# tohinz/multiple-objects-gan

Measured on AMD Instinct MI355X. Metric: images/sec per G+D train step, 256x256 coco-attngan, higher is better.
Workload: dtype f32

## Files before the change

include/mogan_hip.h:

```cpp
#ifndef MOGAN_HIP_H
#define MOGAN_HIP_H

#include <stddef.h>
#include <stdint.h>

#ifdef __cplusplus
extern "C" {
#endif

typedef struct ihipStream_t* hipStream_t;

#define MOGAN_ERR_SHAPE (-1)
#define MOGAN_ERR_LAUNCH (-2)
#define MOGAN_ERR_WS (-3)

#define MOGAN_ACT_NONE 0
#define MOGAN_ACT_RELU 1
#define MOGAN_ACT_LRELU 2
#define MOGAN_ACT_GLU 3
#define MOGAN_ACT_TANH 4
#define MOGAN_ACT_SIGMOID 5

int mogan_abi_version(void);
int mogan_gemm_set_split_target(int blocks);
// ... 34 lines not shown
typedef struct MoganConvDgradArgs {
    const float* dy; long long dy_bstride; const float* w; float* dx; long long dx_bstride;
    const float* relu_of; long long relu_bstride; int accumulate;
    int B, Cin, Hs, Ws, Cout, KH, KW, stride, ph, pw;
} MoganConvDgradArgs;
int mogan_conv2d_affine_fwd_group(int n, const MoganConvFwdArgs* args, void* ws, size_t ws_bytes, hipStream_t stream);
int mogan_conv2d_dgrad_group(int n, const MoganConvDgradArgs* args, void* ws, size_t ws_bytes, hipStream_t stream);
int mogan_conv2d_affine_fwd_ex(const float* x, long long x_bstride, const float* w, const float* scale, const float* shift,
                               float* y, long long y_bstride, float* y2, long long y2_bstride, int msplit, int B, int Cin,
                               int Hs, int Ws, int Cout, int KH, int KW, int stride, int ph, int pw, int relu, void* ws,
                               size_t ws_bytes, hipStream_t stream);
int mogan_conv2d_fwd_ex(const float* x, long long x_bstride, const float* w, float* y, long long y_bstride,
                        const float* relu_of, long long relu_bstride, int accumulate, int B, int Cin, int Hs, int Ws,
                        int Cout, int KH, int KW, int stride, int ph, int pw, void* ws, size_t ws_bytes, hipStream_t stream);
int mogan_conv2d_dgrad_ex(const float* dy, long long dy_bstride, const float* w, float* dx, long long dx_bstride,
                          const float* relu_of, long long relu_bstride, int accumulate, int B, int Cin, int Hs, int Ws,
                          int Cout, int KH, int KW, int stride, int ph, int pw, void* ws, size_t ws_bytes,
                          hipStream_t stream);
int mogan_conv2d_dgrad(const float* dy, const float* w, float* dx, int B, int Cin, int Hs, int Ws, int Cout, int KH,
                       int KW, int stride, int ph, int pw, int up, void* ws, size_t ws_bytes, hipStream_t stream);
size_t mogan_wino_prep_bytes(int B, int Cin, int Hs, int Ws, int Cout, int KH, int KW, int stride, int ph, int pw, int up, int dgrad);
int mogan_wino_prep_group(int n, const float* const* w, void* const* prep, const int* Cout, const int* Cin, const int* dgrad,
                          hipStream_t stream);
size_t mogan_conv_prep_bytes(int B, int Cin, int Hs, int Ws, int Cout, int KH, int KW, int stride, int ph, int pw, int up, int dgrad);
int mogan_conv_prep_group(int n, const float* const* w, void* const* prep, const int* Cout, const int* Cin, const int* KH,
                          const int* dgrad, hipStream_t stream);
int mogan_conv2d_fwd_wp(const float* x, const float* w, const void* wprep, float* y, int B, int Cin, int Hs, int Ws, int Cout, int KH,
                        int KW, int stride, int ph, int pw, int up, void* ws, size_t ws_bytes, hipStream_t stream);
int mogan_conv2d_dgrad_wp(const float* dy, const float* w, const void* wprep, float* dx, int B, int Cin, int Hs, int Ws, int Cout,
                          int KH, int KW, int stride, int ph, int pw, int up, void* ws, size_t ws_bytes, hipStream_t stream);
int mogan_conv2d_wgrad(const float* dy, const float* x, float* dw, int B, int Cin, int Hs, int Ws, int Cout, int KH,
                       int KW, int stride, int ph, int pw, int up, int accumulate, void* ws, size_t ws_bytes,
                       hipStream_t stream);

int mogan_pk_conv_eligible(int B, int Cin, int Hs, int Ws, int Cout, int KH, int KW, int stride, int ph, int pw, int dgrad);
size_t mogan_pk_weight_bytes(int Cout, int Cin, int KH, int KW, int stride, int dgrad);
int mogan_pk_weight_pack(const float* w, void* wpk, int Cout, int Cin, int KH, int KW, int stride, int ph, int pw, int dgrad,
                         hipStream_t stream);
int mogan_pk_weight_pack_both(const float* w, void* wpk_fwd, void* wpk_dgrad, int Cout, int Cin, int KH, int KW, int stride, int ph,
                              int pw, hipStream_t stream);
int mogan_conv2d_fwd_pk(const float* x, const void* wpk, float* y, int B, int Cin, int Hs, int Ws, int Cout, int KH, int KW,
                        int stride, int ph, int pw, void* ws, size_t ws_bytes, hipStream_t stream);
int mogan_conv2d_dgrad_pk(const float* dy, const void* wpk, float* dx, int B, int Cin, int Hs, int Ws, int Cout, int KH, int KW,
                          int stride, int ph, int pw, void* ws, size_t ws_bytes, hipStream_t stream);
int mogan_pk_debug_force(int take_all, int cfg, int split);
int mogan_pk_wgrad_eligible(int B, int Cin, int Hs, int Ws, int Cout, int KH, int KW, int stride, int ph, int pw, size_t ws_bytes);
int mogan_conv2d_wgrad_pk(const float* dy, const float* x, float* dw, int B, int Cin, int Hs, int Ws, int Cout, int KH, int KW,
                          int stride, int ph, int pw, int accumulate, void* ws, size_t ws_bytes, hipStream_t stream);

size_t mogan_pk_panel_bytes(int B, int C, int HW);
int mogan_deep_block_eligible(int B, int Cin, int Hs, int Ws, int Cout, int KH, int KW, int stride, int ph, int pw, int act,
                              int groups);
int mogan_deep_conv_bn_act_fwd(const float* x, const void* xpanel, const void* wpk, const float* gamma, const float* beta,
                               float* rmean, float* rvar, float* y, float* stats, float* z, void* zpanel, int B, int Cin, int Hs,
                               int Ws, int Cout, int KH, int KW, int stride, int ph, int pw, float eps, float momentum, int act,
                               float slope, int groups, void* ws, size_t ws_bytes, hipStream_t stream);
int mogan_deep_conv_bn_act_bwd(const float* dz, const float* y, const float* stats, const float* gamma, const float* beta,
                               const void* wpk_dgrad, float* dy, float* dgamma, float* dbeta, int accumulate, float* dx, int B,
                               int Cin, int Hs, int Ws, int Cout, int KH, int KW, int stride, int ph, int pw, int act, float slope,
                               int groups, void* ws, size_t ws_bytes, hipStream_t stream);

typedef struct MoganPkArgs {
    const void* wpk; const void* panel; float* raw;
    int B, M;
    int Cp, CGp, cg0;
    int PH, PW, outH, outW;
// ... 219 lines not shown
```

multiple-objects-gan_amd/csrc/mogan_dconv2.hip:

```cpp
#include <hip/hip_runtime.h>
#include <stdint.h>
#include <stdlib.h>
#include <algorithm>
#include "../../include/mogan_hip.h"
#include "mogan_internal.h"
#include "mogan_mma.h"

#if MOGAN_X6
#if defined(DCONV2_LAB) && DCONV2_LAB == 9
__device__ unsigned long long g_d2_seg[8];
#define D2_T(var) const unsigned long long var = __builtin_readcyclecounter()
#define D2_ADD(i, a, b) do { if (tid == 0) atomicAdd(&g_d2_seg[i], (b) - (a)); } while (0)
extern "C" int mogan_lab_d2_segments(unsigned long long* out, int reset) {
    if (hipMemcpyFromSymbol(out, HIP_SYMBOL(g_d2_seg), sizeof(g_d2_seg)) != hipSuccess) return -1;
    if (reset) { unsigned long long z[8] = {0}; if (hipMemcpyToSymbol(HIP_SYMBOL(g_d2_seg), z, sizeof(z)) != hipSuccess) return -1; }
    return 0;
}
#else
#define D2_T(var) do {} while (0)
#define D2_ADD(i, a, b) do {} while (0)
#endif
namespace {

typedef float f32x16 __attribute__((ext_vector_type(16)));
typedef float f32x4 __attribute__((ext_vector_type(4)));

__device__ __forceinline__ float ldg1(__amdgpu_buffer_rsrc_t r, unsigned idx) {
    return __builtin_bit_cast(float, __builtin_amdgcn_raw_buffer_load_b32(r, idx * 4u, 0, 0));
}
__device__ __forceinline__ f32x4 ldg4w(__amdgpu_buffer_rsrc_t r, unsigned idx) {
    return __builtin_bit_cast(f32x4, __builtin_amdgcn_raw_buffer_load_b128(r, idx * 4u, 0, 0));
}
#define D2_OOB 0x3FFFFFFFu

struct D2P {
    const float* X; const void* Wp; float* Y; float* ws;
    int B, Cin, Cout, H, W;
    int CinX;
    int OH, OW, pt, pl;
// ... 240 lines not shown
            for (int tt = 0; tt < TM; ++tt)
#pragma unroll
                for (int r = 0; r < 16; ++r) {
                    ybase[(size_t)(tt * 32 + (r & 3) + 8 * (r >> 2)) * plane] = acc[tt][r];
                    acc[tt][r] = 0.f;
                }
        } else {
#pragma unroll
            for (int tt = 0; tt < TM; ++tt)
#pragma unroll
                for (int r = 0; r < 16; ++r) {
                    const int mr = tt * 32 + (r & 3) + 8 * (r >> 2);
                    if (m0 + mr + 4 * h < p.Cout) {
                        float* dst = ybase + (size_t)mr * plane;
                        float v = acc[tt][r];
                        if (addc) v += *dst;
                        *dst = v;
                    }
                    acc[tt][r] = 0.f;
                }
        }
        D2_T(t_e1); D2_ADD(5, t_e0, t_e1);
    }
}

__global__ __launch_bounds__(256) void dconv2_reduce_kernel(const float* __restrict__ ws, float* __restrict__ out, long long n,
                                                            long long slab, int nsplit, int acc) {
    const long long i = (long long)blockIdx.x * 256 + threadIdx.x;
    if (i >= n) return;
    float s = acc ? out[i] : 0.f;
    for (int k = 0; k < nsplit; ++k) s += ws[(size_t)k * slab + i];
    out[i] = s;
}

static inline long long cdiv2(long long a, long long b) { return (a + b - 1) / b; }

template <int KH, int KW, int TM, int NS, int CW, bool S2D>
static int launch2g(D2P& p, hipStream_t st) {
    constexpr int KHW = KH * KW, NPIX = (256 / CW + KH - 1) * (CW + KW - 1);
    constexpr size_t lds = (size_t)NS * 6 * NPIX * 16 + (size_t)TM * 32 * ((size_t)NS * KHW * 6 + 1) * 16;
    static_assert(lds <= 160 * 1024, "LDS budget");
    static bool attr = false;
    if (!attr) {
        if (hipFuncSetAttribute((const void*)dconv2_fwd_kernel<KH, KW, TM, NS, CW, S2D>, hipFuncAttributeMaxDynamicSharedMemorySize,
                                (int)lds) != hipSuccess) return MOGAN_ERR_LAUNCH;
        attr = true;
    }
    dim3 grid((unsigned)cdiv2(p.ntiles, p.tpb), (unsigned)cdiv2(p.Cout, TM * 32), (unsigned)(p.nsplit * p.npar));
    hipLaunchKernelGGL((dconv2_fwd_kernel<KH, KW, TM, NS, CW, S2D>), grid, dim3(512), lds, st, p);
    return 0;
}
template <int KH, int KW, int TM, int NS>
static int launch2(D2P& p, hipStream_t st) {
    return p.tiles_cw == 32 ? launch2g<KH, KW, TM, NS, 32, false>(p, st) : launch2g<KH, KW, TM, NS, 16, false>(p, st);
}

static inline void d2_tile(bool s2d, bool k22, int Cin, int Cout, int& tm, int& ns) {
    tm = 4; long long best = cdiv2(Cout, 128) * 128;
    if (s2d) { tm = 3; best = cdiv2(Cout, 96) * 96; }
    else if (cdiv2(Cout, 96) * 96 < best) { best = cdiv2(Cout, 96) * 96; tm = 3; }
    if (cdiv2(Cout, 64) * 64 < best) { best = cdiv2(Cout, 64) * 64; tm = 2; }
    ns = s2d ? 2 : (k22 && tm <= 3 && Cin % 32 == 0) ? 2 : 1;
}

}
#endif

int mogan_dconv2_prep_group(int n, const float* const* w, void* const* prep, const int* Cout, const int* Cin, const int* dgrad,
// ... 2 lines not shown
    for (int i0 = 0; i0 < n; i0 += D2G_MAX) {
        D2PrepGroup g{};
        g.n = std::min(D2G_MAX, n - i0);
        unsigned end = 0;
        for (int j = 0; j < g.n; ++j) {
            const int i = i0 + j;
            if (!w[i] || !prep[i] || Cout[i] <= 0 || Cin[i] <= 0 || (((uintptr_t)prep[i]) & 15)) return MOGAN_ERR_SHAPE;
            int tm, ns;
            long long rows; int kin, cout1, wmode;
            if (!dgrad[i]) {
                if (Cin[i] % 8) return MOGAN_ERR_SHAPE;
                d2_tile(true, true, 4 * Cin[i], Cout[i], tm, ns);
                rows = Cout[i]; kin = 4 * Cin[i]; cout1 = Cin[i]; wmode = 3;
            } else {
                if (Cout[i] % 16) return MOGAN_ERR_SHAPE;
                d2_tile(false, true, Cout[i], Cin[i], tm, ns);
                rows = 4ll * Cin[i]; kin = Cout[i]; cout1 = Cin[i]; wmode = 2;
            }
            const int nst = kin / (16 * ns);
            g.w[j] = w[i]; g.wp[j] = (uint4*)prep[i]; g.rows[j] = (int)rows; g.Cin[j] = kin; g.NS[j] = ns; g.wmode[j] = wmode; g.Cout1[j] = cout1;
            g.total[j] = (long long)nst * rows * ns * 4 * 2;
            const long long blocks = (g.total[j] + 255) / 256;
            if (blocks <= 0 || (long long)end + blocks > 0x7fffffffLL) return MOGAN_ERR_SHAPE;
            end += (unsigned)blocks; g.end[j] = end;
        }
        hipLaunchKernelGGL(dconv2_wprep_group_kernel, dim3(end), dim3(256), 0, st, g);
    }
    return hipGetLastError() == hipSuccess ? 0 : MOGAN_ERR_LAUNCH;
#else
    return n > 0 ? MOGAN_ERR_SHAPE : 0;
#endif
}

int mogan_dconv2_fwd_try(const float* X, const float* w, int wmode, float* Y, int B, int Cin, int Cout, int H, int W, int OH, int OW,
                         int KH, int KW, int pt, int pl, int yH, int yW, int ys, int npar, int accumulate, void* ws,
                         size_t ws_bytes, hipStream_t st, const void* prep_in, size_t* query) {
#if MOGAN_X6
    constexpr int on = 2;
    if (!on || (on < 2 && (wmode == 3 || (OW % 32) != 0))) return 0;
    const bool s2d = wmode == 3;
    if (s2d) {
        if (KH != 4 || KW != 4 || pt != 1 || pl != 1 || (H & 1) || (W & 1) || OH != H / 2 || OW != W / 2 || (Cin % 8) || npar != 1 ||
            ys != 1) return 0;
        KH = KW = 2; pt = pl = 0;
    }
    const int CinX = Cin;
    if (s2d) Cin *= 4;
    const bool k33 = KH == 3 && KW == 3, k22 = KH == 2 && KW == 2;
    const int cw = (OW % 32) == 0 ? 32 : 16, tr = 256 / cw;
    if (!(k33 || k22) || (OW % cw) || (OH % tr) || (Cin % 16) || Cout < 64 || B <= 0) return 0;
    if ((long long)B * CinX * H * W >= (1ll << 29) || (long long)B * Cout * yH * yW >= (1ll << 30)) return 0;
    const int KHW = KH * KW;
    int tm, ns; d2_tile(s2d, k22, Cin, Cout, tm, ns);
    const int nst = Cin / (16 * ns);
    const long long rows = (long long)npar * Cout;
    const size_t wpb = (size_t)nst * rows * ns * KHW * 6 * 16;
    if (wpb >= (1ull << 31)) return 0;
    const bool owned = wmode == 2 || wmode == 3;
    if (query) { *query = owned ? wpb : 0; return 1; }
    const void* prep = owned ? prep_in : nullptr;
    if (!prep) {
        if (!ws || ws_bytes < wpb + 256) return 0;
        const long long total = (long long)nst * rows * ns * KHW * 2;
        hipLaunchKernelGGL(dconv2_wprep_kernel, dim3((unsigned)((total + 255) / 256)), dim3(256), 0, st, w, (uint4*)ws, (int)rows, Cin,
                           KHW, ns, wmode, s2d ? CinX : Cout, total);
    }
// ... 11 lines not shown
    static int ncu = 0;
    if (!ncu) {
        int dev = 0; hipDeviceProp_t pr;
        if (hipGetDevice(&dev) == hipSuccess && hipGetDeviceProperties(&pr, dev) == hipSuccess) ncu = pr.multiProcessorCount;
        if (ncu <= 0) ncu = 256;
    }
    int nsplit = 1;
    if (tiles < (3 * ncu) / 4 && nst >= 4) nsplit = (int)std::min<long long>(cdiv2(ncu, tiles), nst / 2);
    if (nsplit > 1) {
        const long long fit = (long long)(ws2_bytes / (sizeof(float) * (size_t)y_numel));
        nsplit = fit < 2 ? 1 : (int)std::min<long long>(nsplit, fit);
    }
    p.sps = (int)cdiv2(nst, nsplit); p.nsplit = (int)cdiv2(nst, p.sps);
    p.slab = y_numel; p.ws = (float*)ws2;
    {
        const long long per_group = std::max<long long>(1, ncu / (groups * p.nsplit));
        p.tpb = (int)cdiv2(p.ntiles, std::min<long long>(per_group, p.ntiles));
    }
    if (tiles * p.nsplit > 0x7fffffffLL) return 0;
    mogan_prof_relabel(2);
    int rc = 0;
    if (s2d) {
        if (cw == 32) rc = tm == 3 ? launch2g<2, 2, 3, 2, 32, true>(p, st) : launch2g<2, 2, 2, 2, 32, true>(p, st);
        else rc = tm == 3 ? launch2g<2, 2, 3, 2, 16, true>(p, st) : launch2g<2, 2, 2, 2, 16, true>(p, st);
    } else if (k33) {
        if (tm == 4) rc = launch2<3, 3, 4, 1>(p, st); else if (tm == 3) rc = launch2<3, 3, 3, 1>(p, st); else rc = launch2<3, 3, 2, 1>(p, st);
    } else if (ns == 2) {
        if (tm == 3) rc = launch2<2, 2, 3, 2>(p, st); else rc = launch2<2, 2, 2, 2>(p, st);
    } else {
        if (tm == 4) rc = launch2<2, 2, 4, 1>(p, st); else if (tm == 3) rc = launch2<2, 2, 3, 1>(p, st); else rc = launch2<2, 2, 2, 1>(p, st);
    }
    if (rc) return rc;
    if (p.nsplit > 1)
        hipLaunchKernelGGL(dconv2_reduce_kernel, dim3((unsigned)cdiv2(y_numel, 256)), dim3(256), 0, st, (const float*)ws2, Y, y_numel,
                           y_numel, p.nsplit, accumulate);
    return hipGetLastError() == hipSuccess ? 1 : MOGAN_ERR_LAUNCH;
#else
    return 0;
#endif
}
```

multiple-objects-gan_amd/csrc/mogan_gemm.hip:

```cpp
#include <hip/hip_runtime.h>
#include <stdlib.h>
#include <stdint.h>
#include <stdio.h>
#include <algorithm>
#include <atomic>
#include <mutex>
#include <unordered_map>
#include <vector>
#include "../../include/mogan_hip.h"
#include "mogan_internal.h"
#include "mogan_mma.h"
#ifndef MOGAN_X6_STAGE
#define MOGAN_X6_STAGE 1
#endif
#ifndef MOGAN_DGRAD_PARITY_FAST
#define MOGAN_DGRAD_PARITY_FAST 1
#endif

namespace {

typedef float f32x16 __attribute__((ext_vector_type(16)));
typedef float f32x4 __attribute__((ext_vector_type(4)));

struct FastDiv { uint32_t d, mul, shr; };

static FastDiv make_fd(uint32_t d) {
    FastDiv f; f.d = d ? d : 1; f.mul = 0; f.shr = 0;
    if (f.d > 1) {
        uint32_t l = 0; while ((1u << l) < f.d) ++l;
        uint32_t p = 31 + l;
        f.mul = (uint32_t)(((1ull << p) + f.d - 1) / f.d);
        f.shr = p - 32;
    }
    return f;
}
__device__ __forceinline__ uint32_t fdiv(uint32_t n, const FastDiv& f) {
    return f.d == 1 ? n : (__umulhi(n, f.mul) >> f.shr);
}

enum { CONV_FWD = 0, CONV_DGRAD = 1, CONV_WGRAD = 2, BMM = 3 };

struct GemmP {
    const float* A; const float* B; float* C;
    int M, N, K;
// ... 509 lines not shown
        const unsigned ncls = (MODE == CONV_DGRAD) ? (unsigned)(p.s * p.s) : 1u;
        if (MODE == CONV_DGRAD && ncls > 1 && MOGAN_DGRAD_PARITY_FAST) {
            const unsigned cls = t2 % ncls, t3 = t2 / ncls;
            by = t3 % gy;
            bz = cls * (unsigned)p.nsplit + t3 / gy;
        } else {
            by = t2 % gy; bz = t2 / gy;
        }
    }
    gemm_block<MODE, WM, WN, TM, TN, AVEC>(p, bx, by, bz);
}

constexpr int MAXG = 4;
struct GroupArgs { GemmP p[MAXG]; int tile_end[MAXG]; int gx[MAXG], gy[MAXG]; int nprob; };

template <int MODE, int WM, int WN, int TM, int TN, bool AVEC>
__global__ __launch_bounds__(256) void gemm_group_kernel(const GroupArgs g) {
    const unsigned V = xcd_order(blockIdx.x, gridDim.x);
    int pi = 0;
#pragma unroll
    for (int i = 0; i < MAXG - 1; ++i) if (i + 1 < g.nprob && V >= (unsigned)g.tile_end[i]) pi = i + 1;
    const unsigned local = V - (pi ? (unsigned)g.tile_end[pi - 1] : 0u);
    const unsigned gx = g.gx[pi], gy = g.gy[pi];
    const unsigned bx = local % gx, t2 = local / gx;
    gemm_block<MODE, WM, WN, TM, TN, AVEC>(g.p[pi], bx, t2 % gy, t2 / gy);
}

struct ReduceP {
    long long n, slab, Mcms, cms, ybs, ybs2, mbs;
    int nsplit, acc, msplit, ep_relu;
    float ep_slope;
    const float* ep_scale; const float* ep_shift; const float* mask; float* out2;
};
__global__ __launch_bounds__(256) void splitk_reduce_kernel(const float* __restrict__ ws, float* __restrict__ out,
                                                            const ReduceP q) {
    const long long i = (long long)blockIdx.x * 256 + threadIdx.x;
    if (i >= q.n) return;
    long long img, rem; int m;
    if (q.n < (1ll << 31)) {
        const unsigned iu = (unsigned)i, im = iu / (unsigned)q.Mcms, r = iu - im * (unsigned)q.Mcms;
        img = im; rem = r; m = (int)(r / (unsigned)q.cms);
    } else {
        img = i / q.Mcms; rem = i - img * q.Mcms; m = (int)(rem / q.cms);
    }
    float* dst = out + img * q.ybs + rem;
    if (m >= q.msplit) dst = q.out2 + img * q.ybs2 + (rem - (long long)q.msplit * q.cms);
    const float* p = ws + i;
    float s = 0.f;
    int k = 0;
    for (; k + 8 <= q.nsplit; k += 8) {
        float v[8];
#pragma unroll
        for (int u = 0; u < 8; ++u) v[u] = p[(size_t)(k + u) * q.slab];
#pragma unroll
        for (int u = 0; u < 8; ++u) s += v[u];
    }
    for (; k < q.nsplit; ++k) s += p[(size_t)k * q.slab];
    if (q.mask != nullptr && !(q.mask[img * q.mbs + rem] > 0.f)) s = 0.f;
    if (q.acc) s += *dst;
    if (q.ep_scale != nullptr) {
        s = fmaf(s, q.ep_scale[m], q.ep_shift[m]);
        if (q.ep_relu) s = fmaxf(s, 0.f);
    } else if (q.ep_slope > 0.f) {
        s = s > 0.f ? s : s * q.ep_slope;
    }
    *dst = s;
}

struct Cfg { int wm, wn, tm, tn; };
static const Cfg kCfgs[] = {{2, 2, 2, 2}, {1, 4, 3, 1}, {4, 1, 1, 1}, {1, 4, 1, 1}, {2, 2, 1, 1}, {2, 2, 2, 1}, {2, 2, 1, 2}};
enum { NCFG = 7, NCFG_HEUR = 5 };

template <int MODE, bool AVEC>
static void launch_cfg2(int c, dim3 grid, hipStream_t st, const GemmP& p) {
    switch (c) {
        case 0: hipLaunchKernelGGL((gemm_kernel<MODE, 2, 2, 2, 2, AVEC>), grid, dim3(256), 0, st, p); break;
        case 1: hipLaunchKernelGGL((gemm_kernel<MODE, 1, 4, 3, 1, AVEC>), grid, dim3(256), 0, st, p); break;
        case 2: hipLaunchKernelGGL((gemm_kernel<MODE, 4, 1, 1, 1, AVEC>), grid, dim3(256), 0, st, p); break;
        case 3: hipLaunchKernelGGL((gemm_kernel<MODE, 1, 4, 1, 1, AVEC>), grid, dim3(256), 0, st, p); break;
        case 5: hipLaunchKernelGGL((gemm_kernel<MODE, 2, 2, 2, 1, AVEC>), grid, dim3(256), 0, st, p); break;
        case 6: hipLaunchKernelGGL((gemm_kernel<MODE, 2, 2, 1, 2, AVEC>), grid, dim3(256), 0, st, p); break;
        default: hipLaunchKernelGGL((gemm_kernel<MODE, 2, 2, 1, 1, AVEC>), grid, dim3(256), 0, st, p); break;
    }
}
template <int MODE>
static void launch_cfg(int c, dim3 grid, hipStream_t st, const GemmP& p) {
    if constexpr (MODE == CONV_DGRAD) launch_cfg2<MODE, false>(c, grid, st, p);
    else if (p.avec) launch_cfg2<MODE, true>(c, grid, st, p);
    else launch_cfg2<MODE, false>(c, grid, st, p);
}

template <int MODE, bool AVEC>
static void launch_group2(int c, unsigned nblocks, hipStream_t st, const GroupArgs& g) {
    switch (c) {
        case 0: hipLaunchKernelGGL((gemm_group_kernel<MODE, 2, 2, 2, 2, AVEC>), dim3(nblocks), dim3(256), 0, st, g); break;
        case 5: hipLaunchKernelGGL((gemm_group_kernel<MODE, 2, 2, 2, 1, AVEC>), dim3(nblocks), dim3(256), 0, st, g); break;
        case 6: hipLaunchKernelGGL((gemm_group_kernel<MODE, 2, 2, 1, 2, AVEC>), dim3(nblocks), dim3(256), 0, st, g); break;
        default: hipLaunchKernelGGL((gemm_group_kernel<MODE, 2, 2, 1, 1, AVEC>), dim3(nblocks), dim3(256), 0, st, g); break;
    }
}

static inline long long cdiv(long long a, long long b) { return (a + b - 1) / b; }

static int g_force_cfg = -1, g_force_split = 0;

struct ProfRec { int mode, cfg; double flops; hipEvent_t e0, e1; int M, N, K, nz, nsplit, Cin, Cout, H, W, KH, KW, s, up, Bn; };
static std::vector<ProfRec> g_prof;
static std::mutex g_prof_mu;
static bool g_prof_on = false;

}
void mogan_splitk_reduce_dense(const float* ws, float* out, long long n, int nsplit, int accumulate, hipStream_t st) {
    ReduceP q{};
    q.n = n; q.slab = n; q.nsplit = nsplit; q.acc = accumulate;
    q.Mcms = n; q.cms = n; q.ybs = n; q.msplit = 0x7fffffff;
    hipLaunchKernelGGL(splitk_reduce_kernel, dim3((unsigned)cdiv(n, 256)), dim3(256), 0, st, ws, out, q);
}
int mogan_use_dconv = 1;
static ProfRec g_prof_open; static bool g_prof_open_valid = false;
void mogan_prof_begin(int mode, int cfg, double flops, int M, int N, int K, hipStream_t st) {
    g_prof_open_valid = false;
    if (!g_prof_on) return;
    ProfRec r{}; r.mode = mode; r.cfg = cfg; r.flops = flops; r.M = M; r.N = N; r.K = K; r.nz = 1; r.nsplit = 1;
    hipEventCreate(&r.e0); hipEventCreate(&r.e1); hipEventRecord(r.e0, st);
    g_prof_open = r; g_prof_open_valid = true;
}
void mogan_prof_relabel(int cfg) { if (g_prof_open_valid) g_prof_open.cfg = cfg; }
void mogan_prof_end(int taken, hipStream_t st) {
    if (!g_prof_open_valid) return;
    g_prof_open_valid = false;
    if (!taken) { hipEventDestroy(g_prof_open.e0); hipEventDestroy(g_prof_open.e1); return; }
    hipEventRecord(g_prof_open.e1, st);
    std::lock_guard<std::mutex> lk(g_prof_mu);
    g_prof.push_back(g_prof_open);
}
namespace {

static std::atomic<int> g_split_target{768};
static std::unordered_map<hipStream_t, int> g_stream_target;
static std::mutex g_stream_mu;
static int split_target_of(hipStream_t st) {
    {
        std::lock_guard<std::mutex> lk(g_stream_mu);
        auto it = g_stream_target.find(st);
        if (it != g_stream_target.end()) return it->second;
    }
    return g_split_target.load(std::memory_order_relaxed);
}

// ... 38 lines not shown
    if (g_force_split > 0) nsplit = std::min(g_force_split, ktiles);
    if (nsplit > 1) {
        const long long fit = ws ? (long long)(ws_bytes / (sizeof(float) * (size_t)c_numel)) : 0;
        if (fit < 2) nsplit = 1; else nsplit = (int)std::min<long long>(nsplit, fit);
    }
    int kt_per = (int)cdiv(ktiles, nsplit);
    nsplit = (int)cdiv(ktiles, kt_per);
    p.kchunk = kt_per * 32; p.nsplit = nsplit; p.slab = c_numel; p.ws = (float*)ws;
    if (p.K <= 0) { p.kchunk = 32; p.nsplit = 1; }
    dim3 grid((unsigned)cdiv(p.N, bn), (unsigned)cdiv(p.M, bm), (unsigned)(nz * p.nsplit));
    if (grid.y > 65535 || grid.z > 65535) return MOGAN_ERR_SHAPE;
    ProfRec rec{}; const bool prof = g_prof_on;
    if (prof) {
        rec.mode = mode; rec.cfg = best;
        rec.M = p.M; rec.N = p.N; rec.K = p.K; rec.nz = nz; rec.nsplit = p.nsplit; rec.Cin = p.Cin; rec.Cout = p.Cout;
        rec.H = p.H; rec.W = p.W; rec.KH = p.KH; rec.KW = p.KW; rec.s = p.s; rec.up = p.up; rec.Bn = p.Bn;
        const double ncols = mode == CONV_DGRAD ? (double)p.Bn * p.H * p.W : (double)p.N * nz;
        rec.flops = 2.0 * (double)p.M * ncols * (double)p.K;
        hipEventCreate(&rec.e0); hipEventCreate(&rec.e1);
        hipEventRecord(rec.e0, st);
    }
    switch (mode) {
        case CONV_FWD: launch_cfg<CONV_FWD>(best, grid, st, p); break;
        case CONV_DGRAD: launch_cfg<CONV_DGRAD>(best, grid, st, p); break;
        case CONV_WGRAD: launch_cfg<CONV_WGRAD>(best, grid, st, p); break;
        default: launch_cfg<BMM>(best, grid, st, p); break;
    }
    if (prof) {
        hipEventRecord(rec.e1, st);
        std::lock_guard<std::mutex> lk(g_prof_mu);
        g_prof.push_back(rec);
    }
    if (p.nsplit > 1) {
        const long long nblk = cdiv(c_numel, 256);
        ReduceP q{};
        q.n = c_numel; q.slab = c_numel; q.nsplit = p.nsplit; q.acc = p.accumulate;
        q.Mcms = c_numel; q.cms = c_numel; q.ybs = c_numel; q.msplit = 0x7fffffff;
        if (mode == CONV_FWD || mode == CONV_DGRAD) {
            q.cms = mode == CONV_FWD ? (long long)p.OH * p.OW : (long long)p.H * p.W;
            q.Mcms = (long long)p.M * q.cms; q.ybs = p.ybs; q.msplit = p.msplit; q.out2 = p.C2; q.ybs2 = p.ybs2;
            q.mask = p.mask; q.mbs = p.mbs;
            if (mode == CONV_FWD) { q.ep_scale = p.ep_scale; q.ep_shift = p.ep_shift; q.ep_relu = p.ep_relu; q.ep_slope = p.ep_slope; }
        }
        hipLaunchKernelGGL(splitk_reduce_kernel, dim3((unsigned)nblk), dim3(256), 0, st, (const float*)ws, p.C, q);
    }
    return hipGetLastError() == hipSuccess ? 0 : MOGAN_ERR_LAUNCH;
}

static int g_group_min_tiles = 1600;
static int run_group(int mode, GemmP* ps, const int* nz, int n, hipStream_t st) {
    static const int cand[4] = {0, 5, 6, 4};
    int best = 4; double bestw = 1e300;
    for (int ci = 0; ci < 4; ++ci) {
        const int c = cand[ci];
        const int bm = kCfgs[c].wm * kCfgs[c].tm * 32, bn = kCfgs[c].wn * kCfgs[c].tn * 32;
        double w = 0; long long tiles = 0;
        for (int i = 0; i < n; ++i) {
            const long long t = cdiv(ps[i].M, bm) * cdiv(ps[i].N, bn) * nz[i];
            tiles += t;
            w += (double)t * bm * bn * (double)ps[i].K;
        }
        w *= (bm * bn >= 128 * 128) ? 1.0 : (bm * bn >= 128 * 64 ? 1.04 : 1.10);
        if (tiles < 512) w *= 512.0 / (double)(tiles < 64 ? 64 : tiles);
        if (w < bestw) { bestw = w; best = c; }
    }
    if (g_force_cfg == 0 || g_force_cfg == 4 || g_force_cfg == 5 || g_force_cfg == 6) best = g_force_cfg;
    const int bm = kCfgs[best].wm * kCfgs[best].tm * 32, bn = kCfgs[best].wn * kCfgs[best].tn * 32;
    {
        long long tiles = 0;
        for (int i = 0; i < n; ++i) tiles += cdiv(ps[i].M, bm) * cdiv(ps[i].N, bn) * nz[i];
        if (tiles < g_group_min_tiles && g_force_cfg < 0) return 1;
    }
    GroupArgs g{};
    g.nprob = n;
    long long end = 0; bool avec = true;
    for (int i = 0; i < n; ++i) {
        GemmP& p = ps[i];
// ... 575 lines not shown
```

multiple-objects-gan_amd/csrc/mogan_wino.hip:

```cpp
#include <hip/hip_runtime.h>
#include <stdint.h>
#include <stdlib.h>
#include <algorithm>
#include "../../include/mogan_hip.h"
#include "mogan_internal.h"
#include "mogan_mma.h"

#ifndef MOGAN_WINO5
#define MOGAN_WINO5 1
#endif
#ifndef WGRAD_XCD
#define WGRAD_XCD 1
#endif
#ifndef WGRAD_BLOCKS
#define WGRAD_BLOCKS 256
#endif
#ifndef W5_XCD
#define W5_XCD 1
#endif
#ifndef W5_NT
#define W5_NT 1
#endif

namespace {

typedef float f32x16 __attribute__((ext_vector_type(16)));
typedef float f32x4 __attribute__((ext_vector_type(4)));

constexpr int CK = 8, TROWS = 2, TCOLS = 16, NT = TROWS * TCOLS, BM = 96;
constexpr int XR = 2 * TROWS + 2, XC = 2 * TCOLS + 2, XCP = 36;

__device__ __forceinline__ float ldgx(__amdgpu_buffer_rsrc_t r, unsigned idx, bool ok) {
    return __builtin_bit_cast(float, __builtin_amdgcn_raw_buffer_load_b32(r, ok ? idx * 4u : 0xFFFFFFFCu, 0, 0));
}
__device__ __forceinline__ f32x4 ldgx4(__amdgpu_buffer_rsrc_t r, unsigned idx, bool ok) {
    return __builtin_bit_cast(f32x4, __builtin_amdgcn_raw_buffer_load_b128(r, ok ? idx * 4u : 0xFFFFFFF0u, 0, 0));
}

#if MOGAN_X6
// ... 902 lines not shown
                    for (int a = 0; a < 3; ++a) av[j][kk][a] = Qc[row * LDQ + a * 32 + l31];
                }
            transform_q(Qs + nxt * QSZ);
            load_y(k + 2);
            store_x(Xs + cur * XSZ, 2 * XSZ - cur * XSZ);
            load_x(k + 3);
            transform_v(Xs + nxt * XSZ, Vs + nxt * VSZ);
#pragma unroll
            for (int j = 0; j < 2; ++j)
#pragma unroll
                for (int kk = 0; kk < WCT / 2; ++kk)
#pragma unroll
                    for (int a = 0; a < 3; ++a)
                        acc[j][a] = __builtin_amdgcn_mfma_f32_32x32x2f32(av[j][kk][a], bv[j][kk], acc[j][a], 0, 0, 0);
            __syncthreads();
        }
#endif
    }
    float* out = part + (size_t)sp * 16 * Cout * Cin;
#pragma unroll
    for (int j = 0; j < 2; ++j) {
        const int xi = wave * 2 + j;
#pragma unroll
        for (int a = 0; a < 3; ++a)
#pragma unroll
            for (int r = 0; r < 16; ++r) {
                const int m = m0 + a * 32 + (r & 3) + 8 * (r >> 2) + 4 * h, n = n0 + l31;
                if (m < Cout && n < Cin) out[((size_t)xi * Cout + m) * Cin + n] = acc[j][a][r];
            }
    }
}
}

__global__ __launch_bounds__(64) void wino_wgrad_finish(const float* __restrict__ part, float* __restrict__ dw, int Cout,
                                                         int Cin, int nsplit, int accumulate) {
    const long long i = (long long)blockIdx.x * 64 + threadIdx.x;
    const long long n = (long long)Cout * Cin;
    if (i >= n) return;
    float u[4][4];
#pragma unroll
    for (int a = 0; a < 4; ++a)
#pragma unroll
        for (int b = 0; b < 4; ++b) u[a][b] = 0.f;
    for (int sp = 0; sp < nsplit; ++sp) {
        const float* ps = part + (size_t)sp * 16 * n + i;
#pragma unroll
        for (int a = 0; a < 4; ++a)
#pragma unroll
            for (int b = 0; b < 4; ++b) u[a][b] += ps[(size_t)(a * 4 + b) * n];
    }
    float t[3][4];
#pragma unroll
    for (int b = 0; b < 4; ++b) {
        t[0][b] = u[0][b] + 0.5f * (u[1][b] + u[2][b]);
        t[1][b] = 0.5f * (u[1][b] - u[2][b]);
        t[2][b] = 0.5f * (u[1][b] + u[2][b]) + u[3][b];
    }
    float* d = dw + i * 9;
#pragma unroll
    for (int a = 0; a < 3; ++a) {
        const float g0 = t[a][0] + 0.5f * (t[a][1] + t[a][2]), g1 = 0.5f * (t[a][1] - t[a][2]),
                    g2 = 0.5f * (t[a][1] + t[a][2]) + t[a][3];
        d[a * 3 + 0] = (accumulate ? d[a * 3 + 0] : 0.f) + g0;
        d[a * 3 + 1] = (accumulate ? d[a * 3 + 1] : 0.f) + g1;
        d[a * 3 + 2] = (accumulate ? d[a * 3 + 2] : 0.f) + g2;
    }
}

}

static int g_wino = -1;

int mogan_wino_try(const float* in, const float* w, const void* prep, float* out, const MoganConvShape& g, int dgrad,
                   const float* ep_scale, const float* ep_shift, int ep_relu, void* ws, size_t ws_bytes, hipStream_t st) {
#if MOGAN_X6
    if (g_wino < 0) { const char* e = getenv("MOGAN_WINO"); g_wino = (e && e[0] == '0') ? 0 : 1; }
    const int B = g.B, Cin = g.Cin, H = g.H, W = g.W, Cout = g.Cout, ph = g.ph;
    if (!g_wino || !(g.KH == 3 && g.KW == 3 && g.stride == 1 && ph == g.pw && (ph == 0 || ph == 1) && g.up == 0)) return 0;
    const int Kin = dgrad ? Cout : Cin, Kout = dgrad ? Cin : Cout;
    const int cH = g.OH, cW = g.OW;
    const int iH = dgrad ? cH : H, iW = dgrad ? cW : W, oH = dgrad ? H : cH, oW = dgrad ? W : cW, pad = dgrad ? 2 - ph : ph;
    if (cH < 2 || cW < 2 || (Kin % CK2) || Kin < 32 || Kout < 64) return 0;
    if ((((uintptr_t)out) & 15) != 0) return 0;
// ... 3 lines not shown
    if ((long long)B * Kin * iH * iW >= (1ll << 29) || (long long)Kin * iH * iW >= (1ll << 26) ||
        (long long)B * Kout * oH * oW >= (1ll << 30))
        return 0;
    const size_t u3bytes = (size_t)mbs * 8 * (Kin / CK2) * 18 * 1024 + 18 * 1024;
    if (u3bytes >= (1ull << 31)) return 0;
    if (prep == nullptr && (!ws || u3bytes > ws_bytes)) return 0;
    const uint4* U = prep ? (const uint4*)prep : (const uint4*)ws;
    static int ncu = 0;
    if (!ncu) {
        int dev = 0; hipDeviceProp_t pr;
        if (hipGetDevice(&dev) == hipSuccess && hipGetDeviceProperties(&pr, dev) == hipSuccess) ncu = pr.multiProcessorCount;
        if (ncu <= 0) ncu = 256;
    }
    const int nunit = (int)mbs * 3 * (Kin / CK2);
    if (prep == nullptr)
        hipLaunchKernelGGL(wino3_weight_kernel, dim3((unsigned)((nunit + 3) / 4)), dim3(256), 0, st, w, (uint4*)ws, Cout, Cin, dgrad, nunit);
    if (MOGAN_WINO5 && ep_scale == nullptr && (oH % (2 * TROWS)) == 0 && (oW % (2 * TCOLS)) == 0 && (Kout % BM) == 0) {
        const long long nt5 = (long long)B * tiles_x * tiles_y * mbs;
        mogan_prof_relabel(3);
        hipLaunchKernelGGL(wino5_fwd_kernel, dim3((unsigned)std::min<long long>(nt5, ncu)), dim3(1024), 0, st, in, U, out,
                           Kin, iH, iW, Kout, oH, oW, pad, tiles_x, tiles_y, (int)nt5, (unsigned)(4ull * B * Kin * iH * iW),
                           (unsigned)u3bytes);
        return hipGetLastError() == hipSuccess ? 1 : MOGAN_ERR_LAUNCH;
    }
    const long long ntile = (long long)B * tiles_x * tiles_y * mbs;
    if (ntile >= (1ll << 30)) return 0;
    dim3 grid((unsigned)std::min<long long>(ntile, ncu));
    hipLaunchKernelGGL(wino3_fwd_kernel, grid, dim3(512), 0, st, in, U, out, Kin, iH, iW, Kout, oH, oW, pad, tiles_x,
                       tiles_y, (int)ntile, B, ep_scale, ep_shift, ep_relu, (unsigned)(4ull * B * Kin * iH * iW), (unsigned)u3bytes);
    return hipGetLastError() == hipSuccess ? 1 : MOGAN_ERR_LAUNCH;
#else
    return 0;
#endif
}

int mogan_wino_wgrad_try(const float* dy, const float* x, float* dw, const MoganConvShape& g, int accumulate, void* ws,
                         size_t ws_bytes, hipStream_t st) {
    const int B = g.B, Cin = g.Cin, H = g.H, W = g.W, Cout = g.Cout;
    if (g_wino < 0) { const char* e = getenv("MOGAN_WINO"); g_wino = (e && e[0] == '0') ? 0 : 1; }
    constexpr int wg_on = 1;
    if (!g_wino || !wg_on || !(mogan_is_k33(g) && g.up == 0)) return 0;
    if (Cin < 32 || Cout < 64 || (H % 2) || (W % (2 * WCT)) || (W % 2)) return 0;
    if ((((uintptr_t)dy) & 7) != 0) return 0;
    if ((long long)B * Cin * H * W >= (1ll << 30) || (long long)B * Cout * H * W >= (1ll << 30)) return 0;
    const int nchunk = B * (H / 2) * (W / (2 * WCT));
    const bool rows = Cin % WBN == 0;
    const int cob = (Cout + BM - 1) / BM;
    const int tiles_mn = rows ? cob * (Cin / WBN) * WNP : cob * ((Cin + wg32::WBN - 1) / wg32::WBN);
    const int wg_blocks = rows ? WGRAD_BLOCKS : 192;
    int nsplit = wg_blocks / tiles_mn;
    if (nsplit < 1) nsplit = 1;
    if (nsplit > nchunk / 8) nsplit = nchunk / 8 > 0 ? nchunk / 8 : 1;
    const size_t slab = (size_t)16 * Cout * Cin * sizeof(float);
    if (!ws || ws_bytes < slab) return 0;
    if ((size_t)nsplit * slab > ws_bytes) nsplit = (int)(ws_bytes / slab);
    const int cps = (nchunk + nsplit - 1) / nsplit;
    nsplit = (nchunk + cps - 1) / cps;
    const unsigned yb = (unsigned)(4ull * B * Cout * H * W), xb = (unsigned)(4ull * B * Cin * H * W);
    if (rows) {
        static bool attr = false;
        if (!attr) {
            if (hipFuncSetAttribute((const void*)wino_wgrad_kernel<true>, hipFuncAttributeMaxDynamicSharedMemorySize, (int)WG_LDS) != hipSuccess ||
                hipFuncSetAttribute((const void*)wino_wgrad_kernel<false>, hipFuncAttributeMaxDynamicSharedMemorySize, (int)WG_LDS) != hipSuccess)
                return MOGAN_ERR_LAUNCH;
            attr = true;
        }
        dim3 grid((unsigned)(Cin / WBN), (unsigned)(cob * WNP), (unsigned)nsplit);
        if (Cout % BM == 0)
            hipLaunchKernelGGL(wino_wgrad_kernel<true>, grid, dim3(64 * WNP), WG_LDS, st, dy, x, (float*)ws, Cin, H, W, Cout, nchunk,
                               cps, yb, xb);
        else
            hipLaunchKernelGGL(wino_wgrad_kernel<false>, grid, dim3(64 * WNP), WG_LDS, st, dy, x, (float*)ws, Cin, H, W, Cout, nchunk,
                               cps, yb, xb);
    } else {
        dim3 grid((unsigned)((Cin + wg32::WBN - 1) / wg32::WBN), (unsigned)cob, (unsigned)nsplit);
        hipLaunchKernelGGL(wg32::wino_wgrad_ci32_kernel, grid, dim3(512), 0, st, dy, x, (float*)ws, Cin, H, W, Cout, nchunk, cps, yb, xb);
    }
    const long long n = (long long)Cout * Cin;
    if (wg_on != 2)
    hipLaunchKernelGGL(wino_wgrad_finish, dim3((unsigned)((n + 63) / 64)), dim3(64), 0, st, (const float*)ws, dw, Cout,
                       Cin, nsplit, accumulate);
    return hipGetLastError() == hipSuccess ? 1 : MOGAN_ERR_LAUNCH;
}

size_t mogan_wino_prep_bytes(int B, int Cin, int Hs, int Ws, int Cout, int KH, int KW, int stride, int ph, int pw, int up, int dgrad) {
#if MOGAN_X6
    if (g_wino < 0) { const char* e = getenv("MOGAN_WINO"); g_wino = (e && e[0] == '0') ? 0 : 1; }
    if (!g_wino || !(KH == 3 && KW == 3 && stride == 1 && ph == pw && (ph == 0 || ph == 1) && up == 0)) return 0;
    const int Kin = dgrad ? Cout : Cin, Kout = dgrad ? Cin : Cout;
    const int cH = Hs + 2 * ph - 2, cW = Ws + 2 * pw - 2;
    const int iH = dgrad ? cH : Hs, iW = dgrad ? cW : Ws, oH = dgrad ? Hs : cH, oW = dgrad ? Ws : cW;
    if (cH < 2 || cW < 2 || (Kin % CK2) || Kin < 32 || Kout < 64) return 0;
    const int tiles_x = (oW + 2 * TCOLS - 1) / (2 * TCOLS), tiles_y = (oH + 2 * TROWS - 1) / (2 * TROWS);
    if ((double)oW * oH < 0.7 * (double)tiles_x * 2 * TCOLS * tiles_y * 2 * TROWS) return 0;
    const long long mbs = (Kout + BM - 1) / BM;
    if ((long long)B * Kin * iH * iW >= (1ll << 29) || (long long)Kin * iH * iW >= (1ll << 26) ||
        (long long)B * Kout * oH * oW >= (1ll << 30))
        return 0;
    const size_t u3bytes = (size_t)mbs * 8 * (Kin / CK2) * 18 * 1024 + 18 * 1024;
    return u3bytes < (1ull << 31) ? u3bytes : 0;
#else
    return 0;
#endif
}

int mogan_wino_prep_group(int n, const float* const* w, void* const* prep, const int* Cout, const int* Cin, const int* dgrad,
                          hipStream_t st) {
#if MOGAN_X6
    if (n < 0 || (n > 0 && (!w || !prep || !Cout || !Cin || !dgrad))) return MOGAN_ERR_SHAPE;
    for (int i0 = 0; i0 < n; i0 += WPG_MAX) {
        WinoPrepGroup g{}; unsigned tot = 0;
        g.n = std::min(WPG_MAX, n - i0);
        for (int i = 0; i < g.n; ++i) {
            const int k = i0 + i;
            const int Kin = dgrad[k] ? Cout[k] : Cin[k], Kout = dgrad[k] ? Cin[k] : Cout[k];
// ... 14 lines not shown
```

multiple-objects-gan_amd/hip/lib.py:

```python
import contextlib
import ctypes
import os

import torch

_HERE = os.path.dirname(os.path.dirname(os.path.abspath(__file__)))
LIB_PATH = os.environ.get("MOGAN_LIB") or os.path.join(_HERE, "libmogan_hip.so")

P, I, F, L, Z, D = ctypes.c_void_p, ctypes.c_int, ctypes.c_float, ctypes.c_longlong, ctypes.c_size_t, ctypes.c_double

SIGNATURES = {
    "mogan_abi_version": [],
    "mogan_gemm_set_split_target": [I],
    "mogan_stream_set_split_target": [P, I],
    "mogan_gemm_debug_force": [I, I],
    "mogan_gemm_group_min_tiles": [I],
    "mogan_mfma_form": [],
    "mogan_gemm_tune_set": [I, I, I, I, I, I, I],
    "mogan_gemm_tune_clear": [],
    "mogan_reserve_streams": [ctypes.c_int],
    "mogan_prof_enable": [I],
    "mogan_prof_collect": [P, I],
    "mogan_prof_dump": [ctypes.c_char_p],
    "mogan_conv2d_out_dims": [I, I, I, I, I, I, I, I, P, P],
    "mogan_conv2d_fwd": [P, P, P] + [I] * 11 + [P, Z, P],
    "mogan_logits_head_fwd": [P, P, P, P, I, I, I, P],
    "mogan_logits_head_bwd": [P, P, P, P, P, P, P, I, I, I, I, P],
    "mogan_conv2d_lrelu_fwd": [P, P, P] + [I] * 10 + [F, P, Z, P],
    "mogan_conv2d_affine_fwd": [P, P, P, P, P] + [I] * 11 + [P, Z, P],
    "mogan_affine_relu_bwd_out": [P, P, P, P, I, I, I, P],
    "mogan_conv2d_dgrad": [P, P, P] + [I] * 11 + [P, Z, P],
    "mogan_conv2d_wgrad": [P, P, P] + [I] * 12 + [P, Z, P],
    "mogan_wino_prep_bytes": [I] * 12,
    "mogan_wino_prep_group": [I, P, P, P, P, P, P],
    "mogan_conv_prep_bytes": [I] * 12,
    "mogan_conv_prep_group": [I, P, P, P, P, P, P, P],
    "mogan_conv2d_fwd_wp": [P, P, P, P] + [I] * 11 + [P, Z, P],
    "mogan_conv2d_dgrad_wp": [P, P, P, P] + [I] * 11 + [P, Z, P],
    "mogan_pk_conv_eligible": [I] * 11,
    "mogan_pk_weight_bytes": [I] * 6,
    "mogan_pk_weight_pack": [P, P] + [I] * 8 + [P],
    "mogan_pk_weight_pack_both": [P, P, P] + [I] * 7 + [P],
    "mogan_conv2d_fwd_pk": [P, P, P] + [I] * 10 + [P, Z, P],
    "mogan_conv2d_dgrad_pk": [P, P, P] + [I] * 10 + [P, Z, P],
    "mogan_pk_debug_force": [I, I, I],
    "mogan_pk_wgrad_eligible": [I] * 10 + [Z],
    "mogan_conv2d_wgrad_pk": [P, P, P] + [I] * 11 + [P, Z, P],
    "mogan_pk_panel_bytes": [I, I, I],
    "mogan_deep_block_eligible": [I] * 12,
    "mogan_deep_conv_bn_act_fwd": [P] * 11 + [I] * 10 + [F, F, I, F, I, P, Z, P],
    "mogan_deep_conv_bn_act_bwd": [P] * 9 + [I, P] + [I] * 10 + [I, F, I, P, Z, P],
    "mogan_upconv3x3_ws_bytes": [I, I],
    "mogan_upconv3x3_fwd": [P, P, P, I, I, I, I, I, P, Z, P],
    "mogan_lstm_encoder_fwd": [P] * 11 + [I] * 6 + [P],
    "mogan_upconv3x3_k4": [P, P, I, I, P],
    "mogan_upconv3x3_k4_group": [I, P, P, P, P, P],
    "mogan_upconv3x3_dgrad": [P, P, P, I, I, I, I, I, P, Z, P],
    "mogan_upconv3x3_wgrad": [P, P, P, I, I, I, I, I, I, P, Z, P],
    "mogan_down2_sum": [P, P, I, I, I, P],
    "mogan_bmm": [P, P, P, I, I, I, I] + [L] * 9 + [I, P, Z, P],
    "mogan_bn_ws_bytes": [I, I, I],
    "mogan_bn_stats": [P, I, I, I, F, F, P, P, P, P, P, Z, P],
    "mogan_bn_running_update": [P, P, P, P, I, L, F, F, P],
    "mogan_bn_act_fwd": [P, P, P, P, P, P, P, I, I, I, I, F, P],
    "mogan_bn_act_grouped_eligible": [I, I, I, I],
# ... 246 lines not shown
```

Measured before the change: 443.2.

## Parallelize split-K reductions across threads with LDS tile sums for few-output cases

Adds a shared block-tile reduction helper that assigns 32 outputs per 1024-thread block and spreads the split dimension across threads, summing through LDS. It is used for split-K GEMM, dconv2 and Winograd wgrad finish reductions when outputs are few and splits are many, where the old one-thread-per-output loops left the GPU underused and serialized long loads. The Winograd finish now always uses the tiled path. It also exposes the reductions as C entry points for testing. The cost is extra syncs and LDS traffic, and the tiled path could be slower for mid-sized shapes.

```diff
diff --git a/include/mogan_hip.h b/include/mogan_hip.h
--- a/include/mogan_hip.h
+++ b/include/mogan_hip.h
@@ -90,6 +90,9 @@
 int mogan_conv2d_wgrad(const float* dy, const float* x, float* dw, int B, int Cin, int Hs, int Ws, int Cout, int KH,
                        int KW, int stride, int ph, int pw, int up, int accumulate, void* ws, size_t ws_bytes,
                        hipStream_t stream);
+int mogan_wino_wgrad_finish(const float* part, float* dw, int Cout, int Cin, int nsplit, int accumulate, hipStream_t stream);
+int mogan_splitk_reduce(const float* ws, float* out, long long n, int nsplit, int accumulate, hipStream_t stream);
+int mogan_dconv2_reduce(const float* ws, float* out, long long n, int nsplit, int accumulate, hipStream_t stream);
 
 int mogan_pk_conv_eligible(int B, int Cin, int Hs, int Ws, int Cout, int KH, int KW, int stride, int ph, int pw, int dgrad);
 size_t mogan_pk_weight_bytes(int Cout, int Cin, int KH, int KW, int stride, int dgrad);
diff --git a/multiple-objects-gan_amd/csrc/mogan_dconv2.hip b/multiple-objects-gan_amd/csrc/mogan_dconv2.hip
--- a/multiple-objects-gan_amd/csrc/mogan_dconv2.hip
+++ b/multiple-objects-gan_amd/csrc/mogan_dconv2.hip
@@ -5,6 +5,7 @@
 #include "../../include/mogan_hip.h"
 #include "mogan_internal.h"
 #include "mogan_mma.h"
+#include "mogan_ksum.h"
 
 #if MOGAN_X6
 #if defined(DCONV2_LAB) && DCONV2_LAB == 9
@@ -311,8 +312,22 @@
     for (int k = 0; k < nsplit; ++k) s += ws[(size_t)k * slab + i];
     out[i] = s;
 }
+__global__ __launch_bounds__(ksum::NT) void dconv2_tile_reduce_kernel(const float* __restrict__ ws, float* __restrict__ out,
+                                                                      long long n, long long slab, int nsplit, int acc) {
+    __shared__ float tile[ksum::LDS_FLOATS];
+    const long long i0 = (long long)blockIdx.x * ksum::OB;
+    const int nvalid = n - i0 < ksum::OB ? (int)(n - i0) : ksum::OB, tid = threadIdx.x;
+    const float s = ksum::tile_sum<1>(ws + i0, (size_t)slab, nsplit, nvalid, acc && tid < nvalid ? out[i0 + tid] : 0.f, tile);
+    if (tid < nvalid) out[i0 + tid] = s;
+}
 
 static inline long long cdiv2(long long a, long long b) { return (a + b - 1) / b; }
+static void launch_dconv2_reduce(const float* ws, float* out, long long n, long long slab, int nsplit, int acc, hipStream_t st) {
+    if (ksum::few_outputs_many_splits(n, nsplit))
+        hipLaunchKernelGGL(dconv2_tile_reduce_kernel, dim3(ksum::blocks(n)), dim3(ksum::NT), 0, st, ws, out, n, slab, nsplit, acc);
+    else
+        hipLaunchKernelGGL(dconv2_reduce_kernel, dim3((unsigned)cdiv2(n, 256)), dim3(256), 0, st, ws, out, n, slab, nsplit, acc);
+}
 
 template <int KH, int KW, int TM, int NS, int CW, bool S2D>
 static int launch2g(D2P& p, hipStream_t st) {
@@ -381,6 +396,16 @@
 #endif
 }
 
+int mogan_dconv2_reduce(const float* ws, float* out, long long n, int nsplit, int accumulate, hipStream_t st) {
+#if MOGAN_X6
+    if (!ws || !out || n <= 0 || nsplit <= 0) return MOGAN_ERR_SHAPE;
+    launch_dconv2_reduce(ws, out, n, n, nsplit, accumulate, st);
+    return hipGetLastError() == hipSuccess ? 0 : MOGAN_ERR_LAUNCH;
+#else
+    return MOGAN_ERR_SHAPE;
+#endif
+}
+
 int mogan_dconv2_fwd_try(const float* X, const float* w, int wmode, float* Y, int B, int Cin, int Cout, int H, int W, int OH, int OW,
                          int KH, int KW, int pt, int pl, int yH, int yW, int ys, int npar, int accumulate, void* ws,
                          size_t ws_bytes, hipStream_t st, const void* prep_in, size_t* query) {
@@ -458,8 +483,7 @@
     }
     if (rc) return rc;
     if (p.nsplit > 1)
-        hipLaunchKernelGGL(dconv2_reduce_kernel, dim3((unsigned)cdiv2(y_numel, 256)), dim3(256), 0, st, (const float*)ws2, Y, y_numel,
-                           y_numel, p.nsplit, accumulate);
+        launch_dconv2_reduce((const float*)ws2, Y, y_numel, y_numel, p.nsplit, accumulate, st);
     return hipGetLastError() == hipSuccess ? 1 : MOGAN_ERR_LAUNCH;
 #else
     return 0;
diff --git a/multiple-objects-gan_amd/csrc/mogan_gemm.hip b/multiple-objects-gan_amd/csrc/mogan_gemm.hip
--- a/multiple-objects-gan_amd/csrc/mogan_gemm.hip
+++ b/multiple-objects-gan_amd/csrc/mogan_gemm.hip
@@ -10,6 +10,7 @@
 #include "../../include/mogan_hip.h"
 #include "mogan_internal.h"
 #include "mogan_mma.h"
+#include "mogan_ksum.h"
 #ifndef MOGAN_X6_STAGE
 #define MOGAN_X6_STAGE 1
 #endif
@@ -585,10 +586,7 @@
     float ep_slope;
     const float* ep_scale; const float* ep_shift; const float* mask; float* out2;
 };
-__global__ __launch_bounds__(256) void splitk_reduce_kernel(const float* __restrict__ ws, float* __restrict__ out,
-                                                            const ReduceP q) {
-    const long long i = (long long)blockIdx.x * 256 + threadIdx.x;
-    if (i >= q.n) return;
+__device__ __forceinline__ void reduce_store(const ReduceP& q, float* __restrict__ out, long long i, float s) {
     long long img, rem; int m;
     if (q.n < (1ll << 31)) {
         const unsigned iu = (unsigned)i, im = iu / (unsigned)q.Mcms, r = iu - im * (unsigned)q.Mcms;
@@ -598,17 +596,6 @@
     }
     float* dst = out + img * q.ybs + rem;
     if (m >= q.msplit) dst = q.out2 + img * q.ybs2 + (rem - (long long)q.msplit * q.cms);
-    const float* p = ws + i;
-    float s = 0.f;
-    int k = 0;
-    for (; k + 8 <= q.nsplit; k += 8) {
-        float v[8];
-#pragma unroll
-        for (int u = 0; u < 8; ++u) v[u] = p[(size_t)(k + u) * q.slab];
-#pragma unroll
-        for (int u = 0; u < 8; ++u) s += v[u];
-    }
-    for (; k < q.nsplit; ++k) s += p[(size_t)k * q.slab];
     if (q.mask != nullptr && !(q.mask[img * q.mbs + rem] > 0.f)) s = 0.f;
     if (q.acc) s += *dst;
     if (q.ep_scale != nullptr) {
@@ -618,6 +605,37 @@
         s = s > 0.f ? s : s * q.ep_slope;
     }
     *dst = s;
+}
+__global__ __launch_bounds__(256) void splitk_reduce_kernel(const float* __restrict__ ws, float* __restrict__ out,
+                                                            const ReduceP q) {
+    const long long i = (long long)blockIdx.x * 256 + threadIdx.x;
+    if (i >= q.n) return;
+    const float* p = ws + i;
+    float s = 0.f;
+    int k = 0;
+    for (; k + 8 <= q.nsplit; k += 8) {
+        float v[8];
+#pragma unroll
+        for (int u = 0; u < 8; ++u) v[u] = p[(size_t)(k + u) * q.slab];
+#pragma unroll
+        for (int u = 0; u < 8; ++u) s += v[u];
+    }
+    for (; k < q.nsplit; ++k) s += p[(size_t)k * q.slab];
+    reduce_store(q, out, i, s);
+}
+__global__ __launch_bounds__(ksum::NT) void splitk_tile_reduce_kernel(const float* __restrict__ ws, float* __restrict__ out,
+                                                                      const ReduceP q) {
+    __shared__ float tile[ksum::LDS_FLOATS];
+    const long long i0 = (long long)blockIdx.x * ksum::OB;
+    const int nvalid = q.n - i0 < ksum::OB ? (int)(q.n - i0) : ksum::OB;
+    const float s = ksum::tile_sum<1>(ws + i0, (size_t)q.slab, q.nsplit, nvalid, 0.f, tile);
+    if ((int)threadIdx.x < nvalid) reduce_store(q, out, i0 + threadIdx.x, s);
+}
+static void launch_splitk_reduce(const float* ws, float* out, const ReduceP& q, hipStream_t st) {
+    if (ksum::few_outputs_many_splits(q.n, q.nsplit))
+        hipLaunchKernelGGL(splitk_tile_reduce_kernel, dim3(ksum::blocks(q.n)), dim3(ksum::NT), 0, st, ws, out, q);
+    else
+        hipLaunchKernelGGL(splitk_reduce_kernel, dim3((unsigned)((q.n + 255) / 256)), dim3(256), 0, st, ws, out, q);
 }
 
 struct Cfg { int wm, wn, tm, tn; };
@@ -667,7 +685,12 @@
     ReduceP q{};
     q.n = n; q.slab = n; q.nsplit = nsplit; q.acc = accumulate;
     q.Mcms = n; q.cms = n; q.ybs = n; q.msplit = 0x7fffffff;
-    hipLaunchKernelGGL(splitk_reduce_kernel, dim3((unsigned)cdiv(n, 256)), dim3(256), 0, st, ws, out, q);
+    launch_splitk_reduce(ws, out, q, st);
+}
+int mogan_splitk_reduce(const float* ws, float* out, long long n, int nsplit, int accumulate, hipStream_t st) {
+    if (!ws || !out || n <= 0 || nsplit <= 0) return MOGAN_ERR_SHAPE;
+    mogan_splitk_reduce_dense(ws, out, n, nsplit, accumulate, st);
+    return hipGetLastError() == hipSuccess ? 0 : MOGAN_ERR_LAUNCH;
 }
 int mogan_use_dconv = 1;
 static ProfRec g_prof_open; static bool g_prof_open_valid = false;
@@ -772,7 +795,6 @@
         g_prof.push_back(rec);
     }
     if (p.nsplit > 1) {
-        const long long nblk = cdiv(c_numel, 256);
         ReduceP q{};
         q.n = c_numel; q.slab = c_numel; q.nsplit = p.nsplit; q.acc = p.accumulate;
         q.Mcms = c_numel; q.cms = c_numel; q.ybs = c_numel; q.msplit = 0x7fffffff;
@@ -782,7 +804,7 @@
             q.mask = p.mask; q.mbs = p.mbs;
             if (mode == CONV_FWD) { q.ep_scale = p.ep_scale; q.ep_shift = p.ep_shift; q.ep_relu = p.ep_relu; q.ep_slope = p.ep_slope; }
         }
-        hipLaunchKernelGGL(splitk_reduce_kernel, dim3((unsigned)nblk), dim3(256), 0, st, (const float*)ws, p.C, q);
+        launch_splitk_reduce((const float*)ws, p.C, q, st);
     }
     return hipGetLastError() == hipSuccess ? 0 : MOGAN_ERR_LAUNCH;
 }
diff --git a/multiple-objects-gan_amd/csrc/mogan_ksum.h b/multiple-objects-gan_amd/csrc/mogan_ksum.h
--- /dev/null
+++ b/multiple-objects-gan_amd/csrc/mogan_ksum.h
@@ -0,0 +1,54 @@
+#ifndef MOGAN_KSUM_H
+#define MOGAN_KSUM_H
+#include <hip/hip_runtime.h>
+#include <stddef.h>
+
+namespace ksum {
+
+#ifndef KSUM_NT
+#define KSUM_NT 1024
+#endif
+#ifndef KSUM_LPT
+#define KSUM_LPT 16
+#endif
+constexpr int OB = 32;
+constexpr int NT = KSUM_NT;
+constexpr int LPT = KSUM_LPT;
+constexpr int SWEEP = NT / OB;
+constexpr int ROWS = SWEEP * LPT;
+constexpr int LDS_FLOATS = ROWS * OB;
+static_assert(NT % OB == 0 && NT <= 1024 && LDS_FLOATS * sizeof(float) <= 64 * 1024, "block shape");
+
+static inline bool few_outputs_many_splits(long long n, int nsplit) { return n < 2ll * 1024 * 64 && nsplit >= 16; }
+static inline unsigned blocks(long long n) { return (unsigned)((n + OB - 1) / OB); }
+
+template <int G>
+__device__ __forceinline__ float tile_sum(const float* __restrict__ src, size_t stride, int nrow, int nvalid, float init,
+                                          float* __restrict__ tile) {
+    static_assert(ROWS % G == 0 && G * OB <= NT, "a chain's rows must not straddle passes");
+    const int t = threadIdx.x, c = t % OB, r = t / OB;
+    const int cc = c < nvalid ? c : nvalid - 1;
+    float s = init;
+    for (int r0 = 0; r0 < nrow; r0 += ROWS) {
+        float v[LPT];
+        const float* p = src + (size_t)(r0 + r) * stride + cc;
+#pragma unroll
+        for (int k = 0; k < LPT; ++k) {
+            v[k] = r0 + r + k * SWEEP < nrow ? *p : 0.f;
+            p += (size_t)SWEEP * stride;
+        }
+        if (r0) __syncthreads();
+#pragma unroll
+        for (int k = 0; k < LPT; ++k) tile[(r + k * SWEEP) * OB + c] = v[k];
+        __syncthreads();
+        if (t < G * OB) {
+            const int m = nrow - r0 < ROWS ? nrow - r0 : ROWS;
+#pragma unroll 16
+            for (int row = t / OB; row < m; row += G) s += tile[row * OB + c];
+        }
+    }
+    return s;
+}
+
+}
+#endif
diff --git a/multiple-objects-gan_amd/csrc/mogan_wino.hip b/multiple-objects-gan_amd/csrc/mogan_wino.hip
--- a/multiple-objects-gan_amd/csrc/mogan_wino.hip
+++ b/multiple-objects-gan_amd/csrc/mogan_wino.hip
@@ -5,6 +5,7 @@
 #include "../../include/mogan_hip.h"
 #include "mogan_internal.h"
 #include "mogan_mma.h"
+#include "mogan_ksum.h"
 
 #ifndef MOGAN_WINO5
 #define MOGAN_WINO5 1
@@ -973,23 +974,22 @@
 }
 }
 
-__global__ __launch_bounds__(64) void wino_wgrad_finish(const float* __restrict__ part, float* __restrict__ dw, int Cout,
-                                                         int Cin, int nsplit, int accumulate) {
-    const long long i = (long long)blockIdx.x * 64 + threadIdx.x;
-    const long long n = (long long)Cout * Cin;
-    if (i >= n) return;
+__global__ __launch_bounds__(ksum::NT) void wino_wgrad_finish(const float* __restrict__ part, float* __restrict__ dw, int Cout,
+                                                               int Cin, int nsplit, int accumulate) {
+    __shared__ float tile[ksum::LDS_FLOATS];
+    const long long n = (long long)Cout * Cin, i0 = (long long)blockIdx.x * ksum::OB;
+    const int nvalid = n - i0 < ksum::OB ? (int)(n - i0) : ksum::OB, tid = threadIdx.x;
+    const float s = ksum::tile_sum<16>(part + i0, (size_t)n, 16 * nsplit, nvalid, 0.f, tile);
+    __syncthreads();
+    if (tid < 16 * ksum::OB) tile[tid] = s;
+    __syncthreads();
+    if (tid >= nvalid) return;
+    const long long i = i0 + tid;
     float u[4][4];
 #pragma unroll
     for (int a = 0; a < 4; ++a)
 #pragma unroll
-        for (int b = 0; b < 4; ++b) u[a][b] = 0.f;
-    for (int sp = 0; sp < nsplit; ++sp) {
-        const float* ps = part + (size_t)sp * 16 * n + i;
-#pragma unroll
-        for (int a = 0; a < 4; ++a)
-#pragma unroll
-            for (int b = 0; b < 4; ++b) u[a][b] += ps[(size_t)(a * 4 + b) * n];
-    }
+        for (int b = 0; b < 4; ++b) u[a][b] = tile[(a * 4 + b) * ksum::OB + tid];
     float t[3][4];
 #pragma unroll
     for (int b = 0; b < 4; ++b) {
@@ -1059,6 +1059,11 @@
 #else
     return 0;
 #endif
+}
+
+static void launch_wgrad_finish(const float* part, float* dw, int Cout, int Cin, int nsplit, int accumulate, hipStream_t st) {
+    hipLaunchKernelGGL(wino_wgrad_finish, dim3(ksum::blocks((long long)Cout * Cin)), dim3(ksum::NT), 0, st, part, dw, Cout, Cin,
+                       nsplit, accumulate);
 }
 
 int mogan_wino_wgrad_try(const float* dy, const float* x, float* dw, const MoganConvShape& g, int accumulate, void* ws,
@@ -1103,11 +1108,17 @@
         dim3 grid((unsigned)((Cin + wg32::WBN - 1) / wg32::WBN), (unsigned)cob, (unsigned)nsplit);
         hipLaunchKernelGGL(wg32::wino_wgrad_ci32_kernel, grid, dim3(512), 0, st, dy, x, (float*)ws, Cin, H, W, Cout, nchunk, cps, yb, xb);
     }
-    const long long n = (long long)Cout * Cin;
     if (wg_on != 2)
-    hipLaunchKernelGGL(wino_wgrad_finish, dim3((unsigned)((n + 63) / 64)), dim3(64), 0, st, (const float*)ws, dw, Cout,
-                       Cin, nsplit, accumulate);
+    launch_wgrad_finish((const float*)ws, dw, Cout, Cin, nsplit, accumulate, st);
     return hipGetLastError() == hipSuccess ? 1 : MOGAN_ERR_LAUNCH;
+}
+
+int mogan_wino_wgrad_finish(const float* part, float* dw, int Cout, int Cin, int nsplit, int accumulate, hipStream_t st) {
+    if (!part || !dw || Cout <= 0 || Cin <= 0 || nsplit <= 0 || (long long)Cout * Cin >= (1ll << 31) ||
+        nsplit > 0x7fffffff / 16)
+        return MOGAN_ERR_SHAPE;
+    launch_wgrad_finish(part, dw, Cout, Cin, nsplit, accumulate, st);
+    return hipGetLastError() == hipSuccess ? 0 : MOGAN_ERR_LAUNCH;
 }
 
 size_t mogan_wino_prep_bytes(int B, int Cin, int Hs, int Ws, int Cout, int KH, int KW, int stride, int ph, int pw, int up, int dgrad) {
diff --git a/multiple-objects-gan_amd/hip/lib.py b/multiple-objects-gan_amd/hip/lib.py
--- a/multiple-objects-gan_amd/hip/lib.py
+++ b/multiple-objects-gan_amd/hip/lib.py
@@ -31,6 +31,9 @@
     "mogan_affine_relu_bwd_out": [P, P, P, P, I, I, I, P],
     "mogan_conv2d_dgrad": [P, P, P] + [I] * 11 + [P, Z, P],
     "mogan_conv2d_wgrad": [P, P, P] + [I] * 12 + [P, Z, P],
+    "mogan_wino_wgrad_finish": [P, P, I, I, I, I, P],
+    "mogan_splitk_reduce": [P, P, L, I, I, P],
+    "mogan_dconv2_reduce": [P, P, L, I, I, P],
     "mogan_wino_prep_bytes": [I] * 12,
     "mogan_wino_prep_group": [I, P, P, P, P, P, P],
     "mogan_conv_prep_bytes": [I] * 12,
```

Result: no change. 443.0 (-0.1%).
